# cmusatyalab/mega-nerf-viewer

Hardware: AMD Instinct MI355X
Metric: Mrays/sec at 1920x1080 on depth-10 SH-9 N3Tree; max|dRGBA| vs ref (higher is better)
Workload: dtype f32; 1 GPU; cfg2: depth-10 SH9 shell N3Tree (1,499,569 chunks), 1920x1080, 16-pose orbit per step x 4 laps; kernel=accel, partition=none, reserved_cus=0, march_streams=1, root_period=0, full=False

## Files before the change

### mega-nerf-viewer_amd/csrc/mnv_device.h

```cpp
#pragma once

#include <hip/hip_runtime.h>
#include <stdint.h>

#pragma clang fp contract(off)

namespace mnv {

struct __attribute__((aligned(16))) CamBlock {
    float fx, fy, cx, cy;
    float c2w[12];
    float cen[3];
    float pad;
};

struct FrameParams {
    CamBlock cam;
    int32_t x0, y0, tw, th;
    float offset[3], scale[3];
    float step_size, sigma_thresh, stop_thresh, background_brightness;
    float render_bbox[6];
    int32_t basis_min, basis_max;
    int32_t render_depth;
    int32_t rot_enabled;
    float rot_k[3], rot_cos, rot_sin;
    float *rgba;
    uint8_t *rgba8;
    const float *tmax_px;
    const uint8_t *rgba8_init;
};

__device__ __forceinline__ float frame_tmax(const FrameParams &P, int64_t p) { return P.tmax_px ? P.tmax_px[p] : 1e9f; }

struct MarchParams : FrameParams {
    const uint16_t *data;
    const int32_t *child;
    const int16_t *sample_counts;
    int32_t data_dim, basis_dim, format, capacity;
    int32_t max_depth, max_sample_count;
    float *split_track;
    float *sample_track;
    int32_t *visited;
    int32_t track_visit;
    int32_t N;
};

__device__ static const uint64_t kExp2fTab[32] = {
    0x3ff0000000000000ULL, 0x3fefd9b0d3158574ULL, 0x3fefb5586cf9890fULL, 0x3fef9301d0125b51ULL,
    0x3fef72b83c7d517bULL, 0x3fef54873168b9aaULL, 0x3fef387a6e756238ULL, 0x3fef1e9df51fdee1ULL,
    0x3fef06fe0a31b715ULL, 0x3feef1a7373aa9cbULL, 0x3feedea64c123422ULL, 0x3feece086061892dULL,
    0x3feebfdad5362a27ULL, 0x3feeb42b569d4f82ULL, 0x3feeab07dd485429ULL, 0x3feea47eb03a5585ULL,
    0x3feea09e667f3bcdULL, 0x3fee9f75e8ec5f74ULL, 0x3feea11473eb0187ULL, 0x3feea589994cce13ULL,
    0x3feeace5422aa0dbULL, 0x3feeb737b0cdc5e5ULL, 0x3feec49182a3f090ULL, 0x3feed503b23e255dULL,
    0x3feee89f995ad3adULL, 0x3feeff76f2fb5e47ULL, 0x3fef199bdd85529cULL, 0x3fef3720dcef9069ULL,
    0x3fef5818dcfba487ULL, 0x3fef7c97337b9b5fULL, 0x3fefa4afa2a490daULL, 0x3fefd0765b6e4540ULL,
};

__device__ __forceinline__ void load_exp_table(uint64_t *lds_tab) {
    if (threadIdx.x < 32) lds_tab[threadIdx.x] = kExp2fTab[threadIdx.x];
    __syncthreads();
}

__device__ __forceinline__ double expf_poly(double r, double c0, double c1, double c2) {
    double z, y;
    asm("v_fma_f64 %0, %1, %2, %3" : "=v"(z) : "s"(c0), "v"(r), "v"(c1));
    asm("v_fma_f64 %0, %1, %2, %3" : "=v"(y) : "v"(z), "v"(r), "s"(c2));
    return __builtin_fma(y, r, 1.0);
}

__device__ __forceinline__ float exact_expf(float x, const uint64_t *tab) {
    const uint32_t ix = __float_as_uint(x);
    const uint32_t abstop = (ix >> 20) & 0x7ffu;
    if (abstop >= 0x42bu) {
        if (ix == 0xff800000u) return 0.0f;
        if (abstop >= 0x7f8u) return x + x;
        if (x > 0x1.62e42ep6f) return __uint_as_float(0x7f800000u);
        if (x < -0x1.9fe368p6f) return 0.0f;
    }
    constexpr double N = 32.0;
    constexpr double InvLn2N = 0x1.71547652b82fep+0 * N;
    constexpr double SHIFT = 0x1.8p+52;
    constexpr double C0 = 0x1.c6af84b912394p-5 / N / N / N;
    constexpr double C1 = 0x1.ebfce50fac4f3p-3 / N / N;
    constexpr double C2 = 0x1.62e42ff0c52d6p-1 / N;
    const double xd = (double)x;
    double z = InvLn2N * xd;
    double kd = z + SHIFT;
    const uint64_t ki = (uint64_t)__double_as_longlong(kd);
    kd -= SHIFT;
    const double r = z - kd;
    uint64_t t = tab[ki & 31u];
    t += ki << 47;
    const double s = __longlong_as_double((long long)t);
    double y = expf_poly(r, C0, C1, C2);
    y = y * s;
    return (float)y;
}

__device__ __forceinline__ bool exact_expf_core_in_range(uint32_t abs_bits) { return abs_bits < 0x42b00000u; }
__device__ __forceinline__ float exact_expf_core(float x, const uint64_t *tab) {
    constexpr double N = 32.0;
    constexpr double InvLn2N = 0x1.71547652b82fep+0 * N;
    constexpr double SHIFT = 0x1.8p+52;
    constexpr double C0 = 0x1.c6af84b912394p-5 / N / N / N;
    constexpr double C1 = 0x1.ebfce50fac4f3p-3 / N / N;
    constexpr double C2 = 0x1.62e42ff0c52d6p-1 / N;
    const double xd = (double)x;
    double z = InvLn2N * xd;
    double kd = z + SHIFT;
    const uint64_t ki = (uint64_t)__double_as_longlong(kd);
    kd -= SHIFT;
    const double r = z - kd;
    uint64_t t = tab[ki & 31u];
    t += ki << 47;
    const double s = __longlong_as_double((long long)t);
    double y = expf_poly(r, C0, C1, C2);
    y = y * s;
    return (float)y;
}

__device__ __forceinline__ float exact_expf_select(float x, const uint64_t *tab) {
    constexpr double N = 32.0;
    constexpr double InvLn2N = 0x1.71547652b82fep+0 * N;
    constexpr double SHIFT = 0x1.8p+52;
    constexpr double C0 = 0x1.c6af84b912394p-5 / N / N / N;
    constexpr double C1 = 0x1.ebfce50fac4f3p-3 / N / N;
    constexpr double C2 = 0x1.62e42ff0c52d6p-1 / N;
    const float xc = __builtin_amdgcn_fmed3f(x, -128.f, 128.f);
    const double xd = (double)xc;
    double z = InvLn2N * xd;
    double kd = z + SHIFT;
    const uint64_t ki = (uint64_t)__double_as_longlong(kd);
    kd -= SHIFT;
    const double r = z - kd;
    uint64_t t = tab[ki & 31u];
    t += ki << 47;
    const double s = __longlong_as_double((long long)t);
    double y = expf_poly(r, C0, C1, C2);
    y = y * s;
    float res = (float)y;
    const uint32_t ix = __float_as_uint(x);
    const uint32_t abstop = (ix >> 20) & 0x7ffu;
    const bool big = abstop >= 0x42bu;
    res = (big && x < -0x1.9fe368p6f) ? 0.0f : res;
    res = (big && x > 0x1.62e42ep6f) ? __uint_as_float(0x7f800000u) : res;
    res = (big && abstop >= 0x7f8u) ? x + x : res;
    res = ix == 0xff800000u ? 0.0f : res;
    return res;
}

template <bool FAST>
__device__ __forceinline__ float colour_sigmoid(float w, float tmp, const uint64_t *s_exp) {
    if constexpr (FAST) {
        const float x = tmp * -1.44269504088896341f;
        const bool big = x > 96.f;
        const float e = __builtin_amdgcn_exp2f(big ? x - 64.f : x);
        const float den = __builtin_ldexpf((big ? 0x1p-64f : 1.f) + e, -32);
        return __builtin_ldexpf(w * __builtin_amdgcn_rcpf(den), big ? -96 : -32);
    } else {
        return w / (1.f + exact_expf(-tmp, s_exp));
    }
}

__device__ __forceinline__ float half_bits_to_float(uint16_t h) {
    _Float16 v;
    __builtin_memcpy(&v, &h, 2);
    return (float)v;
}

template <int BASIS>
__device__ __forceinline__ void sh_basis(const float vdir[3], float *out) {
    out[0] = (float)0.28209479177387814;
    if constexpr (BASIS >= 4) {
        const float x = vdir[0], y = vdir[1], z = vdir[2];
        const float xx = x * x, yy = y * y, zz = z * z;
        const float xy = x * y, yz = y * z, xz = x * z;
        if constexpr (BASIS >= 25) {
            out[16] = (float)(2.5033429417967046 * xy * (xx - yy));
            out[17] = (float)(-1.7701307697799304 * yz * (3 * xx - yy));
            out[18] = (float)(0.9461746957575601 * xy * (7 * zz - 1.f));
            out[19] = (float)(-0.6690465435572892 * yz * (7 * zz - 3.f));
            out[20] = (float)(0.10578554691520431 * (zz * (35 * zz - 30) + 3));
            out[21] = (float)(-0.6690465435572892 * xz * (7 * zz - 3));
            out[22] = (float)(0.47308734787878004 * (xx - yy) * (7 * zz - 1.f));
            out[23] = (float)(-1.7701307697799304 * xz * (xx - 3 * yy));
            out[24] = (float)(0.6258357354491761 * (xx * (xx - 3 * yy) - yy * (3 * xx - yy)));
        }
        if constexpr (BASIS >= 16) {
            out[9] = (float)(-0.5900435899266435 * y * (3 * xx - yy));
            out[10] = (float)(2.890611442640554 * xy * z);
            out[11] = (float)(-0.4570457994644658 * y * (4 * zz - xx - yy));
            out[12] = (float)(0.3731763325901154 * z * (2 * zz - 3 * xx - 3 * yy));
            out[13] = (float)(-0.4570457994644658 * x * (4 * zz - xx - yy));
            out[14] = (float)(1.445305721320277 * z * (xx - yy));
            out[15] = (float)(-0.5900435899266435 * x * (xx - 3 * yy));
        }
        if constexpr (BASIS >= 9) {
            out[4] = (float)(1.0925484305920792 * xy);
            out[5] = (float)(-1.0925484305920792 * yz);
            out[6] = (float)(0.31539156525252005 * (2.0 * zz - xx - yy));
            out[7] = (float)(-1.0925484305920792 * xz);
            out[8] = (float)(0.5462742152960396 * (xx - yy));
        }
        out[1] = (float)(-0.4886025119029199 * y);
        out[2] = (float)(0.4886025119029199 * z);
        out[3] = (float)(-0.4886025119029199 * x);
    }
}

__device__ __forceinline__ void world_ray_dirs(const FrameParams &P, const CamBlock &C, int ix, int iy, float true_dir[3], float vdir[3]) {
    const float *m = C.c2w;
    const float xyz0 = (ix + 0.5f - C.cx) / C.fx, xyz1 = -(iy + 0.5f - C.cy) / C.fy, xyz2 = -1.0f;
    true_dir[0] = m[0] * xyz0 + m[3] * xyz1 + m[6] * xyz2;
    true_dir[1] = m[1] * xyz0 + m[4] * xyz1 + m[7] * xyz2;
    true_dir[2] = m[2] * xyz0 + m[5] * xyz1 + m[8] * xyz2;
    const float inv = 1.f / sqrtf(true_dir[0] * true_dir[0] + true_dir[1] * true_dir[1] + true_dir[2] * true_dir[2]);
    for (int i = 0; i < 3; ++i) {
        true_dir[i] *= inv;
        vdir[i] = true_dir[i];
    }
    if (P.rot_enabled) {
        const float *k = P.rot_k;
        float cross[3];
        cross[0] = k[1] * vdir[2] - k[2] * vdir[1];
        cross[1] = k[2] * vdir[0] - k[0] * vdir[2];
        cross[2] = k[0] * vdir[1] - k[1] * vdir[0];
        const float dot = k[0] * vdir[0] + k[1] * vdir[1] + k[2] * vdir[2];
        for (int i = 0; i < 3; ++i)
            vdir[i] = (float)((double)(vdir[i] * P.rot_cos + cross[i] * P.rot_sin) + (double)(k[i] * dot) * (1.0 - (double)P.rot_cos));
    }
}

template <int NB>
struct RaySetup {
    float dir[3];
    float invdir[3];
    float basis[NB];
    float delta_scale;
    float tmin, tmax;
    bool in_bbox;
};

template <int BASIS>
__device__ __forceinline__ void setup_ray(const FrameParams &P, const CamBlock &C, int ix, int iy,
                                          RaySetup<(BASIS > 0 ? BASIS : 1)> &r, float t_max = 1e9f) {
    const float xyz0 = (ix + 0.5f - C.cx) / C.fx;
    const float xyz1 = -(iy + 0.5f - C.cy) / C.fy;
    const float xyz2 = -1.0f;
    const float *m = C.c2w;
    float dir[3];
    dir[0] = m[0] * xyz0 + m[3] * xyz1 + m[6] * xyz2;
    dir[1] = m[1] * xyz0 + m[4] * xyz1 + m[7] * xyz2;
    dir[2] = m[2] * xyz0 + m[5] * xyz1 + m[8] * xyz2;
    const float invnorm = 1.f / sqrtf(dir[0] * dir[0] + dir[1] * dir[1] + dir[2] * dir[2]);
    dir[0] *= invnorm;
    dir[1] *= invnorm;
    dir[2] *= invnorm;

    float vdir[3] = {dir[0], dir[1], dir[2]};
    if (P.rot_enabled) {
        const float *k = P.rot_k;
        float cross[3];
        cross[0] = k[1] * vdir[2] - k[2] * vdir[1];
        cross[1] = k[2] * vdir[0] - k[0] * vdir[2];
        cross[2] = k[0] * vdir[1] - k[1] * vdir[0];
        const float dot = k[0] * vdir[0] + k[1] * vdir[1] + k[2] * vdir[2];
#pragma unroll
        for (int i = 0; i < 3; ++i) {
            vdir[i] = (float)((double)(vdir[i] * P.rot_cos + cross[i] * P.rot_sin) +
                              (double)(k[i] * dot) * (1.0 - (double)P.rot_cos));
        }
    }

    dir[0] *= P.scale[0];
    dir[1] *= P.scale[1];
    dir[2] *= P.scale[2];
    const float delta_scale = 1.f / sqrtf(dir[0] * dir[0] + dir[1] * dir[1] + dir[2] * dir[2]);
    dir[0] *= delta_scale;
    dir[1] *= delta_scale;
    dir[2] *= delta_scale;
    r.delta_scale = delta_scale;
    const float tmax_bg = t_max / delta_scale;

    float tmin = 0.0f, tmax = 1e4f;
#pragma unroll
    for (int i = 0; i < 3; ++i) {
        r.dir[i] = dir[i];
        r.invdir[i] = (float)(1.0 / ((double)dir[i] + 1e-9));
        const double inv = (double)r.invdir[i];
        const float t1 = (float)(((double)P.render_bbox[i] + 1e-6 - (double)C.cen[i]) * inv);
        const float t2 = (float)(((double)P.render_bbox[i + 3] - 1e-6 - (double)C.cen[i]) * inv);
        tmin = fmaxf(tmin, fminf(t1, t2));
        tmax = fminf(tmax, fmaxf(t1, t2));
    }
    tmax = fminf(tmax, tmax_bg);
    r.tmin = tmin;
    r.tmax = tmax;
    r.in_bbox = !(tmax < 0 || tmin > tmax);

    constexpr int NB = (BASIS > 0 ? BASIS : 1);
    if constexpr (BASIS > 0) {
        sh_basis<BASIS>(vdir, r.basis);
#pragma unroll
        for (int i = 0; i < NB; ++i)
            if (i < P.basis_min || i > P.basis_max) r.basis[i] = 0.f;
    } else {
        r.basis[0] = 0.f;
    }
}

template <int BASIS>
__device__ __forceinline__ void setup_ray_dir(const FrameParams &P, const float (&cen)[3], float (&dir)[3],
                                              RaySetup<(BASIS > 0 ? BASIS : 1)> &r, float t_max) {
    const float invnorm = 1.f / sqrtf(dir[0] * dir[0] + dir[1] * dir[1] + dir[2] * dir[2]);
    dir[0] *= invnorm;
    dir[1] *= invnorm;
    dir[2] *= invnorm;

    float vdir[3] = {dir[0], dir[1], dir[2]};
    if (P.rot_enabled) {
        const float *k = P.rot_k;
        float cross[3];
        cross[0] = k[1] * vdir[2] - k[2] * vdir[1];
        cross[1] = k[2] * vdir[0] - k[0] * vdir[2];
        cross[2] = k[0] * vdir[1] - k[1] * vdir[0];
        const float dot = k[0] * vdir[0] + k[1] * vdir[1] + k[2] * vdir[2];
#pragma unroll
        for (int i = 0; i < 3; ++i) {
            vdir[i] = (float)((double)(vdir[i] * P.rot_cos + cross[i] * P.rot_sin) +
                              (double)(k[i] * dot) * (1.0 - (double)P.rot_cos));
        }
    }

    dir[0] *= P.scale[0];
    dir[1] *= P.scale[1];
    dir[2] *= P.scale[2];
    const float delta_scale = 1.f / sqrtf(dir[0] * dir[0] + dir[1] * dir[1] + dir[2] * dir[2]);
    dir[0] *= delta_scale;
    dir[1] *= delta_scale;
    dir[2] *= delta_scale;
    r.delta_scale = delta_scale;
    const float tmax_bg = t_max / delta_scale;

    float tmin = 0.0f, tmax = 1e4f;
#pragma unroll
    for (int i = 0; i < 3; ++i) {
        r.dir[i] = dir[i];
        r.invdir[i] = (float)(1.0 / ((double)dir[i] + 1e-9));
        const double inv = (double)r.invdir[i];
        const float t1 = (float)(((double)P.render_bbox[i] + 1e-6 - (double)cen[i]) * inv);
        const float t2 = (float)(((double)P.render_bbox[i + 3] - 1e-6 - (double)cen[i]) * inv);
        tmin = fmaxf(tmin, fminf(t1, t2));
        tmax = fminf(tmax, fmaxf(t1, t2));
    }
    tmax = fminf(tmax, tmax_bg);
    r.tmin = tmin;
    r.tmax = tmax;
    r.in_bbox = !(tmax < 0 || tmin > tmax);

    constexpr int NB = (BASIS > 0 ? BASIS : 1);
    if constexpr (BASIS > 0) {
        sh_basis<BASIS>(vdir, r.basis);
#pragma unroll
        for (int i = 0; i < NB; ++i)
            if (i < P.basis_min || i > P.basis_max) r.basis[i] = 0.f;
    } else {
        r.basis[0] = 0.f;
    }
}

template <int BASIS, typename F>
__device__ __forceinline__ float sh_channel(const float *b, F coef, int off) {
    float tmp = b[0] * coef(off);
    if constexpr (BASIS >= 25) {
        tmp += b[16] * coef(off + 16) + b[17] * coef(off + 17) + b[18] * coef(off + 18) +
               b[19] * coef(off + 19) + b[20] * coef(off + 20) + b[21] * coef(off + 21) +
               b[22] * coef(off + 22) + b[23] * coef(off + 23) + b[24] * coef(off + 24);
    }
    if constexpr (BASIS >= 16) {
        tmp += b[9] * coef(off + 9) + b[10] * coef(off + 10) + b[11] * coef(off + 11) +
               b[12] * coef(off + 12) + b[13] * coef(off + 13) + b[14] * coef(off + 14) +
               b[15] * coef(off + 15);
    }
    if constexpr (BASIS >= 9) {
        tmp += b[4] * coef(off + 4) + b[5] * coef(off + 5) + b[6] * coef(off + 6) + b[7] * coef(off + 7) +
               b[8] * coef(off + 8);
    }
    if constexpr (BASIS >= 4) {
        tmp += b[1] * coef(off + 1) + b[2] * coef(off + 2) + b[3] * coef(off + 3);
    }
    return tmp;
}

__device__ __forceinline__ float half_mul(uint32_t word, bool hi, float b) {
    float r;
    if (hi) asm("v_fma_mix_f32 %0, %1, %2, neg(0) op_sel:[1,0,0] op_sel_hi:[1,0,0]" : "=v"(r) : "v"(word), "v"(b));
    else asm("v_fma_mix_f32 %0, %1, %2, neg(0) op_sel_hi:[1,0,0]" : "=v"(r) : "v"(word), "v"(b));
    return r;
}

template <int BASIS, typename W>
__device__ __forceinline__ float sh_channel_mix(const float *b, W word, int off) {
    auto p = [&](int k) -> float { return half_mul(word((off + k) >> 1), ((off + k) & 1) != 0, b[k]); };
    float tmp = p(0);
    if constexpr (BASIS >= 25) {
        tmp += p(16) + p(17) + p(18) + p(19) + p(20) + p(21) + p(22) + p(23) + p(24);
    }
    if constexpr (BASIS >= 16) {
        tmp += p(9) + p(10) + p(11) + p(12) + p(13) + p(14) + p(15);
    }
    if constexpr (BASIS >= 9) {
        tmp += p(4) + p(5) + p(6) + p(7) + p(8);
    }
    if constexpr (BASIS >= 4) {
        tmp += p(1) + p(2) + p(3);
    }
    return tmp;
}

__device__ __forceinline__ uint32_t pack_u8(float v) {
    const float s = v * 255.f;
    if (!(s > 0.f)) return 0u;
    if (s >= 255.f) return 255u;
    return (uint32_t)s;
}

__device__ __forceinline__ void composite_and_write(const FrameParams &P, int64_t p, float o0, float o1,
                                                    float o2, float o3) {
    const float nalpha = 1.f - o3;
    if (P.rgba8_init) {
        const uint32_t px = reinterpret_cast<const uint32_t *>(P.rgba8_init)[p];
        o0 += (float)(int)(px & 0xffu) / 255.f * nalpha;
        o1 += (float)(int)((px >> 8) & 0xffu) / 255.f * nalpha;
        o2 += (float)(int)((px >> 16) & 0xffu) / 255.f * nalpha;
    } else {
        const float remain = P.background_brightness * nalpha;
        o0 += remain;
        o1 += remain;
        o2 += remain;
    }
    if (P.rgba) reinterpret_cast<float4 *>(P.rgba)[p] = make_float4(o0, o1, o2, o3);
    if (P.rgba8)
        reinterpret_cast<uint32_t *>(P.rgba8)[p] =
            pack_u8(o0) | (pack_u8(o1) << 8) | (pack_u8(o2) << 16) | (255u << 24);
}

}
```

### mega-nerf-viewer_amd/csrc/mnv_march_accel_kernel.h

```cpp
#pragma once

#include "mnv_march_diag.h"

#pragma clang fp contract(off)

namespace mnv {

enum : int { kShapeGeneric = 0, kShapeL3G9 = 1, kShapeL3G9Recs = 2 };
constexpr int kShapeLdsLevel = 3, kShapeGrid2Level = 9;

template <int BASIS, int BLOCK, int MODE ,
          bool BRICK = false ,
          bool RAYS = false ,
          int SHAPE = kShapeGeneric >
#if defined(MNV_NUM_VGPR) && defined(MNV_NUM_SGPR)
#define MNV_EXTRA_KERNEL_ATTR __attribute__((amdgpu_num_vgpr(MNV_NUM_VGPR), amdgpu_num_sgpr(MNV_NUM_SGPR)))
#elif defined(MNV_NUM_VGPR)
#define MNV_EXTRA_KERNEL_ATTR __attribute__((amdgpu_num_vgpr(MNV_NUM_VGPR)))
#else
#define MNV_EXTRA_KERNEL_ATTR
#endif
__global__ __launch_bounds__(BLOCK, (MODE == 2 || MODE == 3) ? MNV_TRACK_WAVES : RAYS ? MNV_RAY_WAVES : MNV_MIN_WAVES) MNV_EXTRA_KERNEL_ATTR void march_accel_kernel(const LaunchBlock<RAYS> K) {
    extern __shared__ __attribute__((aligned(16))) uint32_t s_mem[];
    uint64_t *s_exp = reinterpret_cast<uint64_t *>(s_mem);
    constexpr int NB = BASIS > 0 ? BASIS : 1;
    auto depth_mode = [&]() -> bool {
        if constexpr (MODE == 0 || MODE == 4) return false;
        else if constexpr (MODE == 5) return true;
        else return K.P.render_depth != 0;
    };
    constexpr int MAPW = BASIS >= 16 ? BLOCK : 0;
    uint32_t *s_map = s_mem + 64;
    float *s_ray = reinterpret_cast<float *>(s_mem + 64 + MAPW);
    constexpr int RAY_ROWS = NB + 2 + ((MODE == 2 || MODE == 3) ? 1 : 0);
    uint32_t *s_grid = s_mem + 64 + MAPW + RAY_ROWS * BLOCK;
    constexpr int CHAN_BYTES = chan_bytes_for(BASIS);
    constexpr int ROW_BYTES = row_bytes_pow2(BASIS);
    const FrameParams &P = K.P;
    const AccelView &A = K.A;

    static_assert(SHAPE == kShapeGeneric || (BRICK && !RAYS && (MODE == 0 || MODE == 4)), "fixed lookup shapes: plain colour frames on inline cell words only");
    constexpr bool FIXED = SHAPE != kShapeGeneric;
    const int LL = FIXED ? kShapeLdsLevel : K.lds_level;
    const int cells = 1 << (3 * LL);
    if (threadIdx.x < 32) s_exp[threadIdx.x] = kExp2fTab[threadIdx.x];
    if (LL == A.grid_level) {
        for (int i = threadIdx.x; i < cells; i += BLOCK) s_grid[i] = A.grid[i];
    } else {
        for (int i = threadIdx.x; i < cells; i += BLOCK) {
            const int G = 1 << LL;
            const int iz = i & (G - 1), iy = (i >> LL) & (G - 1), ix = i >> (2 * LL);
            uint32_t chunk = 0, word = 0;
            for (int l = 1; l <= LL; ++l) {
                const int s = LL - l;
                const int cidx = (((ix >> s) & 1) << 2) | (((iy >> s) & 1) << 1) | ((iz >> s) & 1);
                word = A.nodes[(int64_t)chunk * 8 + cidx];
                if (word & kLeafBit) break;
                chunk = word;
            }
            s_grid[i] = word;
        }
    }
    __syncthreads();

    const int lane = threadIdx.x & 63;
    const int Lq = FIXED ? 23 : A.max_depth;
    const float qscale = FIXED ? 8388608.f : __uint_as_float((uint32_t)(127 + Lq) << 23);
    const int sh1 = Lq - LL;
    const int L2 = FIXED ? kShapeGrid2Level : A.grid2_level;
    const int sh2 = Lq - L2;
    const int shg = Lq - A.grid_level;
    float *my_ray = s_ray + threadIdx.x;
    float *wave_ray = s_ray + (threadIdx.x & ~63);

    const CamBlock *__restrict__ Cp = K.cams;
    float cen0 = 0.f, cen1 = 0.f, cen2 = 0.f;
    if constexpr (!RAYS) {
        cen0 = Cp->cen[0];
        cen1 = Cp->cen[1];
        cen2 = Cp->cen[2];
    }
    float t = 0.f, T = 1.f, o0 = 0.f, o1 = 0.f, o2 = 0.f;
    float dir0 = 0.f, dir1 = 0.f, dir2 = 0.f, inv0 = 0.f, inv1 = 0.f, inv2 = 0.f, tmax = 0.f;
    bool alive = false;
    float max_weight = -1.f, max_sample_weight = -1.f, sp_prio = 0.f, sa_prio = 0.f;
    int32_t sp_vox = -1, sa_vox = -1;
    int32_t ns = 0;
    [[maybe_unused]] float sp_t = -1.f, sa_t = -1.f;
    [[maybe_unused]] auto leaf_at = [&](float tw, uint32_t &word, uint32_t &v, float &dt) {
        float pos[3];
        uint32_t q[3];
        pos[0] = cen0 + tw * dir0;
        pos[1] = cen1 + tw * dir1;
        pos[2] = cen2 + tw * dir2;
#pragma unroll
        for (int i = 0; i < 3; ++i) {
            pos[i] = __builtin_amdgcn_fmed3f(pos[i], 0.f, 1.f - 1e-6f);
            q[i] = (uint32_t)(pos[i] * qscale);
        }
        word = s_grid[((((q[0] >> sh1) << LL) | (q[1] >> sh1)) << LL) | (q[2] >> sh1)];
        int src = 0;
        v = 0;
        if (!(word & kLeafBit)) word = descend_to_leaf(A, q, word, sh1, sh2, L2, LL, src, v);
        if (src == 0) v = A.grid_vox[((((q[0] >> shg) << A.grid_level) + (q[1] >> shg)) << A.grid_level) + (q[2] >> shg)];
        else if (src == 1) v = A.grid2_vox[v];
        const int depth = (int)((word >> 16) & 0x7fu);
        const float sc = __uint_as_float((uint32_t)(127 + depth) << 23), inv_cube = __uint_as_float((uint32_t)(127 - depth) << 23);
        const float invd[3] = {inv0, inv1, inv2};
        float tu = 1e4f;
#pragma unroll
        for (int i = 0; i < 3; ++i) {
            const float x = __builtin_amdgcn_fractf(pos[i] * sc);
            const float t1 = -x * invd[i];
            const float t2 = t1 + invd[i];
            tu = fminf(tu, fmaxf(t1, t2));
        }
        dt = tu * inv_cube + P.step_size;
    };
    [[maybe_unused]] auto resolve_fallbacks = [&]() {
        if constexpr (MODE == 2 || MODE == 3) {
            const bool want_split = max_weight == -1.f && sp_t >= 0.f, want_sample = K.sample_counts && max_sample_weight == -1.f && sa_t >= 0.f;
            uint32_t word = 0, v = 0;
            float dt = 0.f;
            if (want_split) {
                leaf_at(sp_t, word, v, dt);
                sp_vox = (int32_t)v;
                sp_prio = (float)((word >> 16) & 0x7fu);
            }
            if (want_sample) {
                if (!(want_split && sa_t == sp_t)) leaf_at(sa_t, word, v, dt);
                const int16_t sc_last = K.sample_counts[v];
                if (sc_last < K.max_sample_count) {
                    sa_vox = (int32_t)v;
                    sa_prio = (float)sc_last;
                } else {
                    float tw = my_ray[(NB + 2) * BLOCK];
                    while (tw < t) {
                        leaf_at(tw, word, v, dt);
                        if (!(half_bits_to_float((uint16_t)word) > P.sigma_thresh)) {
                            const int16_t c = K.sample_counts[v];
                            if (c < K.max_sample_count) {
                                sa_vox = (int32_t)v;
                                sa_prio = (float)c;
                            }
                        }
                        tw += dt;
                    }
                }
            }
        }
    };
    auto write_trackers = [&](uint32_t p) {
        resolve_fallbacks();
        if constexpr (MODE == 3) K.num_samples[p] = (int16_t)ns;
        if constexpr (MODE == 2 || MODE == 3) {
            if (K.split_track) {
                K.split_track[(int64_t)p * 3 + 0] = sp_prio;
                K.split_track[(int64_t)p * 3 + 1] = sp_vox < 0 ? -1.f : (float)(sp_vox >> 3);
                K.split_track[(int64_t)p * 3 + 2] = sp_vox < 0 ? -1.f : (float)(sp_vox & 7);
            }
            if (K.sample_track) {
                K.sample_track[(int64_t)p * 3 + 0] = sa_prio;
                K.sample_track[(int64_t)p * 3 + 1] = sa_vox < 0 ? -1.f : (float)(sa_vox >> 3);
                K.sample_track[(int64_t)p * 3 + 2] = sa_vox < 0 ? -1.f : (float)(sa_vox & 7);
            }
        }
    };

    int fin = 0;
    auto flush_finished = [&]() {
        if (fin != 0) {
            float a;
            if (fin == 3) {
                o0 = o1 = o2 = 0.f;
                a = depth_mode() ? 1.f : 0.f;
            } else if (fin == 1) {
                a = 1.f - T;
                if (depth_mode()) {
                    o0 = o1 = o2 = fminf(o0 * 0.3f, 1.0f);
                    a = 1.f;
                }
            } else {
                if (depth_mode()) o0 = o1 = o2 = fminf(o0 * 0.3f, 1.0f);
                const float sc = 1.f / (1.f - T);
                o0 *= sc;
                o1 *= sc;
                o2 *= sc;
                a = 1.f;
            }
            const uint32_t p = __float_as_uint(my_ray[(NB + 1) * BLOCK]);
            if constexpr (MODE != 3) composite_and_write(P, (int64_t)p, o0, o1, o2, a);
            write_trackers(p);
            fin = 0;
        }
    };

    const uint32_t home = blockIdx.x % kNumQueues;
    uint32_t qsel = 0;
    bool drained = false;
    uint32_t frame = 0;
    uint32_t pix_base = 0;

    MarchProbe<MODE, RAYS, BLOCK> probe(K, lane);
    probe.wave_begin();

    for (;;) {
        const uint64_t idle = __ballot(!alive);
        const int n_idle = __popcll(idle);
        probe.count(kCountOuterIter, true);
        probe.iteration();
        if (!drained && n_idle >= K.refill_min) {
            flush_finished();
            if (qsel >= kNumQueues) {
                drained = true;
            } else {
            const uint32_t q = (home + qsel) % kNumQueues;
            const uint32_t begin = K.band_begin[q] * 64u, span = (K.band_begin[q + 1] - K.band_begin[q]) * 64u;
            const uint32_t grab = (uint32_t)n_idle;
            uint32_t off = 0;
            if (lane == 0) off = atomicAdd(&K.queue[q * 16], grab);
            off = __builtin_amdgcn_readfirstlane(off);
            if (span == 0 || (uint64_t)off >= (uint64_t)span * K.n_frames) {
                ++qsel;
                continue;
            }
            uint32_t f = 0;
            if (K.n_frames > 1) {
                f = off / span;
                off -= f * span;
                if (f != frame) {
                    frame = f;
                    Cp = K.cams + f;
                    cen0 = Cp->cen[0];
                    cen1 = Cp->cen[1];
                    cen2 = Cp->cen[2];
                    pix_base = f * K.frame_stride_px;
                }
            }
            const uint32_t base = begin + off, end = begin + span;
            probe.tile_grabbed(f, base);
            if (!alive) {
                const uint32_t rank = __builtin_amdgcn_mbcnt_hi((uint32_t)(idle >> 32), __builtin_amdgcn_mbcnt_lo((uint32_t)idle, 0u));
                const uint32_t id = base + rank;
                if (rank < grab && id < end) {
                    int bx, by;
                    probe.count(kCountRefill, true);
                    uint32_t pix;
                    if (ray_pixel(K, id, bx, by, pix)) {
                        pix += pix_base;
                        if constexpr (MODE == 2 || MODE == 3) {
                            max_weight = max_sample_weight = -1.f;
                            sp_prio = (float)(K.max_depth + 1);
                            sa_prio = (float)(K.max_sample_count + 1);
                            sp_vox = sa_vox = -1;
                            sp_t = sa_t = -1.f;
                        }
                        if constexpr (MODE == 3) ns = K.num_samples[pix];
                        RaySetup<NB> r;
                        if constexpr (RAYS) {
                            const float *__restrict__ ro = K.ray_origins + (int64_t)pix * 3, *__restrict__ rd = K.ray_dirs + (int64_t)pix * 3;
                            const float w0 = ro[0], w1 = ro[1], w2 = ro[2];
                            float d[3] = {rd[0], rd[1], rd[2]};
                            const float len2 = d[0] * d[0] + d[1] * d[1] + d[2] * d[2];
                            const bool valid = len2 > 0.f && len2 < __builtin_inff() && (w0 - w0) + (w1 - w1) + (w2 - w2) == 0.f;
                            const float p0 = P.scale[0] * w0, p1 = P.scale[1] * w1, p2 = P.scale[2] * w2;
                            const float cen[3] = {P.offset[0] + p0, P.offset[1] + p1, P.offset[2] + p2};
                            setup_ray_dir<(BASIS > 0 ? BASIS : 0)>(P, cen, d, r, frame_tmax(P, pix));
                            r.in_bbox = r.in_bbox && valid;
                            cen0 = cen[0];
                            cen1 = cen[1];
                            cen2 = cen[2];
                        } else {
                            setup_ray<(BASIS > 0 ? BASIS : 0)>(P, *Cp, P.x0 + bx, P.y0 + by, r, frame_tmax(P, pix));
                        }
                        if constexpr (BASIS == 0)
                            r.basis[0] = (0 < P.basis_min || 0 > P.basis_max) ? 0.f : (float)0.28209479177387814;
                        o0 = o1 = o2 = 0.f;
                        if (r.in_bbox) {
                            alive = true;
                            t = r.tmin;
                            T = 1.f;
                            tmax = r.tmax;
                            dir0 = r.dir[0]; dir1 = r.dir[1]; dir2 = r.dir[2];
                            inv0 = r.invdir[0]; inv1 = r.invdir[1]; inv2 = r.invdir[2];
                            if constexpr (MODE == 3) {
                                float true_dir[3], vdir[3];
                                world_ray_dirs(P, *Cp, P.x0 + bx, P.y0 + by, true_dir, vdir);
#pragma unroll
                                for (int k = 0; k < 3; ++k) {
                                    my_ray[k * BLOCK] = true_dir[k];
                                    my_ray[(3 + k) * BLOCK] = vdir[k];
                                }
                            } else {
#pragma unroll
                                for (int k = 0; k < NB; ++k) my_ray[k * BLOCK] = r.basis[k];
                            }
                            my_ray[NB * BLOCK] = r.delta_scale;
                            my_ray[(NB + 1) * BLOCK] = __uint_as_float(pix);
                            if constexpr (MODE == 2 || MODE == 3) my_ray[(NB + 2) * BLOCK] = r.tmin;
                        } else {
                            my_ray[(NB + 1) * BLOCK] = __uint_as_float(pix);
                            fin = 3;
                        }
                    }
                }
            }
            }
        }
        if (__ballot(alive) == 0) {
            probe.tile_done();
            if (drained) {
                flush_finished();
                break;
            }
            continue;
        }
        bool dense = false;
        [[maybe_unused]] bool cand = false;
        [[maybe_unused]] float sigma_held = 0.f;
        float delta_t = 0.f, weight = 0.f, att = 1.f;
        uint32_t vox = 0;
        [[maybe_unused]] bool track_leaf = false;
        [[maybe_unused]] int track_depth = 0;
        [[maybe_unused]] auto track_update = [&]() {
            if constexpr (MODE == 2 || MODE == 3) {
                if (track_leaf) {
                    if (dense) {
                        if (track_depth < K.max_depth && weight > max_weight) {
                            sp_vox = (int32_t)vox;
                            sp_prio = (float)track_depth;
                            max_weight = weight;
                        }
                        if (K.sample_counts && weight > max_sample_weight) {
                            const int16_t sc = K.sample_counts[vox];
                            if (sc < K.max_sample_count) {
                                sa_vox = (int32_t)vox;
                                sa_prio = (float)sc;
                                max_sample_weight = weight;
                            }
                        }
                    } else {
                        if (max_weight == -1.f && track_depth < K.max_depth) sp_t = t;
                        if (max_sample_weight == -1.f) sa_t = t;
                    }
                }
            }
        };
        probe.step_begin();
        if (alive) {
            if (!(t < tmax)) {
                fin = 1;
                alive = false;
            } else {
                probe.count(kCountMarchStep, true);
                float pos[3];
                uint32_t q[3];
                pos[0] = cen0 + t * dir0;
                pos[1] = cen1 + t * dir1;
                pos[2] = cen2 + t * dir2;
#pragma unroll
                for (int i = 0; i < 3; ++i) {
                    pos[i] = __builtin_amdgcn_fmed3f(pos[i], 0.f, 1.f - 1e-6f);
                    q[i] = (uint32_t)(pos[i] * qscale);
                }
                uint32_t word = s_grid[((((q[0] >> sh1) << LL) | (q[1] >> sh1)) << LL) | (q[2] >> sh1)];
                int src = 0;
                if (!(word & kLeafBit)) {
                    int sh = sh1;
                    if (L2 > LL) {
                        const int LB = L2 - 2;
                        uint32_t g = q[0] >> (sh2 + 2);
                        g = (g << LB) | (q[1] >> (sh2 + 2));
                        g = (g << LB) | (q[2] >> (sh2 + 2));
                        g = (g << 2) | __builtin_amdgcn_ubfe(q[0], (uint32_t)sh2, 2u);
                        g = (g << 2) | __builtin_amdgcn_ubfe(q[1], (uint32_t)sh2, 2u);
                        vox = (g << 2) | __builtin_amdgcn_ubfe(q[2], (uint32_t)sh2, 2u);
                        if constexpr (BRICK) word = A.grid2i[vox];
                        else word = A.grid2[vox];
                        probe.touch(kLinesGrid2, (uint64_t)vox * 4);
                        src = 1;
                        sh = sh2;
                        if constexpr ((kShadow & 8) != 0) shadow_load(A.grid2_vox + vox);
                        if constexpr (BRICK) {
                            if (!(word & kLeafBit)) {
                                uint32_t s1 = __builtin_amdgcn_ubfe(q[0], (uint32_t)(sh2 - 1), 1u);
                                s1 = (s1 << 1) | __builtin_amdgcn_ubfe(q[1], (uint32_t)(sh2 - 1), 1u);
                                s1 = (s1 << 1) | __builtin_amdgcn_ubfe(q[2], (uint32_t)(sh2 - 1), 1u);
                                if (word & kInlineBit) {
                                    vox = (((word & ((1u << kInlineMaskShift) - 1u)) + A.inline_base) << 3) | s1;
                                    cand = ((word >> (kInlineMaskShift + s1)) & 1u) != 0u;
                                    word = kLeafBit | ((uint32_t)(L2 + 1) << 16);
                                    src = 2;
                                }
                            }
                            if (SHAPE != kShapeL3G9 && !(word & kLeafBit) && (SHAPE == kShapeL3G9Recs || A.recs != nullptr)) {
                                probe.count(kCountNodeLoad, true);
                                uint32_t s1 = __builtin_amdgcn_ubfe(q[0], (uint32_t)(sh2 - 1), 1u), s2 = __builtin_amdgcn_ubfe(q[0], (uint32_t)(sh2 - 2), 1u);
                                s1 = (s1 << 1) | __builtin_amdgcn_ubfe(q[1], (uint32_t)(sh2 - 1), 1u);
                                s2 = (s2 << 1) | __builtin_amdgcn_ubfe(q[1], (uint32_t)(sh2 - 2), 1u);
                                s1 = (s1 << 1) | __builtin_amdgcn_ubfe(q[2], (uint32_t)(sh2 - 1), 1u);
                                s2 = (s2 << 1) | __builtin_amdgcn_ubfe(q[2], (uint32_t)(sh2 - 2), 1u);
                                const uint2 e = A.recs[(int64_t)word * 8 + s1];
                                probe.touch(kLinesRecs, ((uint64_t)word * 8 + s1) * 8);
                                if constexpr ((kShadow & 64) != 0) shadow_load(K.shadow_recs + ((int64_t)word * 8 + s1));
                                const uint32_t code = __builtin_amdgcn_ubfe(e.y, s2 << 1, 2u);
                                vox = code == 1u ? ((word << 3) | s1) : ((e.x << 3) | s2);
                                cand = code == 3u;
                                word = code != 0u ? (kLeafBit | ((uint32_t)(L2 + 2 - (code == 1u ? 1 : 0)) << 16)) : word;
                                src = 2;
                            }
                        }
                    }
                    while (!(word & kLeafBit)) {
                        probe.count(kCountNodeLoad, true);
                        --sh;
                        uint32_t v = (word << 1) | __builtin_amdgcn_ubfe(q[0], (uint32_t)sh, 1u);
                        v = (v << 1) | __builtin_amdgcn_ubfe(q[1], (uint32_t)sh, 1u);
                        vox = (v << 1) | __builtin_amdgcn_ubfe(q[2], (uint32_t)sh, 1u);
                        word = A.nodes[vox];
                        probe.touch(kLinesNodes, (uint64_t)vox * 4);
                        src = 2;
                        if constexpr ((kShadow & 16) != 0) shadow_load(K.shadow_nodes + vox);
                    }
                }
                if constexpr (BRICK && MODE == 3) {
                    if (cand) {
                        word = A.nodes[vox];
                        cand = false;
                    }
                }
                probe.template phase_end<kPhaseLookup>();
                const int depth = (int)((word >> 16) & 0x7fu);
                const float sc = __uint_as_float((uint32_t)(127 + depth) << 23);
                const float inv_cube = __uint_as_float((uint32_t)(127 - depth) << 23);
                float tu = 1e4f;
                const float invd[3] = {inv0, inv1, inv2};
#pragma unroll
                for (int i = 0; i < 3; ++i) {
                    const float x = __builtin_amdgcn_fractf(pos[i] * sc);
                    const float t1 = -x * invd[i];
                    const float t2 = t1 + invd[i];
                    tu = fminf(tu, fmaxf(t1, t2));
                }
                delta_t = tu * inv_cube + P.step_size;
                const float sigma = half_bits_to_float((uint16_t)word);
                const bool is_dense = sigma > P.sigma_thresh && !probe.ablate(2);
                bool need_vox = is_dense;
                if constexpr (MODE == 2 || MODE == 3) need_vox = is_dense || cand || K.visited != nullptr;
                if (need_vox) {
                    if (src == 0) {
                        const uint32_t gc = ((((q[0] >> shg) << A.grid_level) + (q[1] >> shg)) << A.grid_level) + (q[2] >> shg);
                        vox = A.grid_vox[gc];
                        probe.touch(kLinesGridVox, (uint64_t)gc * 4);
                    } else if (src == 1) {
                        probe.touch(kLinesGrid2Vox, (uint64_t)vox * 4);
                        vox = A.grid2_vox[vox];
                    }
                }
                if constexpr (MODE == 2 || MODE == 3) {
                    if (K.visited && __hip_atomic_load(&K.visited[vox >> 3], __ATOMIC_RELAXED, __HIP_MEMORY_SCOPE_AGENT) == 0) K.visited[vox >> 3] = 1;
                }
                if constexpr (BRICK && MODE != 3) {
                    dense = (is_dense || cand) && !probe.ablate(2);
                    sigma_held = sigma;
                } else if (is_dense) {
                    dense = true;
                    att = exact_expf(-delta_t * my_ray[NB * BLOCK] * sigma, s_exp);
                    weight = T * (1.f - att);
                }
                if constexpr (MODE == 2 || MODE == 3) {
                    track_leaf = true;
                    track_depth = depth;
                    if constexpr (!(BRICK && MODE == 2)) track_update();
                }
                if constexpr (MODE == 3) {
                    if (is_dense && ns < K.max_guided_samples) {
                        const uint32_t p = __float_as_uint(my_ray[(NB + 1) * BLOCK]);
                        float *row = K.samples + ((int64_t)p * K.max_guided_samples + ns) * K.samples_dim;
                        const float tz0 = t * dir0 / P.scale[0], tz1 = t * dir1 / P.scale[1], tz2 = t * dir2 / P.scale[2];
                        const float z = sqrtf(tz0 * tz0 + tz1 * tz1 + tz2 * tz2);
                        const float *m = Cp->c2w;
                        const float wx = m[9] + my_ray[0 * BLOCK] * z, wy = m[10] + my_ray[1 * BLOCK] * z, wz = m[11] + my_ray[2 * BLOCK] * z;
                        row[0] = z;
                        row[1] = wx;
                        row[2] = wy;
                        row[3] = wz;
                        if (K.need_viewdir) {
                            row[4] = my_ray[3 * BLOCK];
                            row[5] = my_ray[4 * BLOCK];
                            row[6] = my_ray[5 * BLOCK];
                            if (K.appearance_embedding != -1) row[7] = (float)K.appearance_embedding;
                        } else if (K.appearance_embedding != -1) {
                            row[4] = (float)K.appearance_embedding;
                        }
                        const int g1 = (int)fmaxf(fminf((wy - K.min_position[1]) / K.range[1] * (float)K.grid_dim[0], (float)K.grid_dim[0] - 1.0f), 0.0f);
                        const int g2 = (int)fmaxf(fminf((wz - K.min_position[2]) / K.range[2] * (float)K.grid_dim[1], (float)K.grid_dim[1] - 1.0f), 0.0f);
                        K.cluster_indices[(int64_t)p * K.max_guided_samples + ns] = (int16_t)(g1 * K.grid_dim[1] + g2);
                        ns += 1;
                    }
                }
            }
        }
        probe.template phase_end<kPhaseStep>();
        const uint64_t dense_mask = __ballot(dense);
        if (dense_mask != 0) {
            probe.count(kCountDense, dense);
            [[maybe_unused]] auto settle = [&](uint32_t row_sigma_bits) {
                const float sg = cand ? half_bits_to_float((uint16_t)row_sigma_bits) : sigma_held;
                if (sg > P.sigma_thresh) {
                    att = exact_expf(-delta_t * my_ray[NB * BLOCK] * sg, s_exp);
                    weight = T * (1.f - att);
                } else {
                    dense = false;
                }
            };
            [[maybe_unused]] auto settle_from_memory = [&]() {
                if constexpr (BRICK) {
                    if (dense && cand) probe.touch(kLinesRows, (uint64_t)vox * A.row_bytes + A.sigma_off);
                    if (dense) settle(cand ? (uint32_t)*reinterpret_cast<const uint16_t *>(A.rows + (int64_t)vox * A.row_bytes + A.sigma_off) : 0u);
                }
            };
            if constexpr (MODE == 3) {
            } else if (depth_mode()) {
                settle_from_memory();
                if (dense) o0 += weight * t;
            } else if (probe.ablate(1)) {
                settle_from_memory();
            } else if constexpr (BASIS >= 16) {
                const int n_dense = __popcll(dense_mask);
                const int rank = (int)__builtin_amdgcn_mbcnt_hi((uint32_t)(dense_mask >> 32), __builtin_amdgcn_mbcnt_lo((uint32_t)dense_mask, 0u));
                uint32_t *map = s_map + (threadIdx.x & ~63);
                if (dense) map[rank] = (uint32_t)lane;
                __builtin_amdgcn_wave_barrier();
                const int my_s = lane / 3, my_c = lane - 3 * my_s;
                for (int base = 0; base < n_dense; base += 21) {
                    const int smp = base + my_s;
                    const bool task = my_s < 21 && smp < n_dense;
                    probe.count(kCountColourPass, task);
                    const int owner = task ? (int)map[smp] : lane;
                    const float w = lane_read(weight, owner);
                    uint32_t vx = lane_read(vox, owner);
                    if (probe.ablate(4)) vx &= 0xffffu;
                    float b[NB];
#pragma unroll
                    for (int k = 0; k < NB; ++k) b[k] = wave_ray[k * BLOCK + owner];
                    float v = 0.f;
                    if (task) {
                        constexpr int NW = CHAN_BYTES / 4;
                        ChanWords<NW> cw;
                        cw = *reinterpret_cast<const ChanWords<NW> *>(A.rows + (int64_t)vx * ROW_BYTES + my_c * CHAN_BYTES);
                        const float tmp = sh_channel_mix<BASIS>(b, [&](int j) -> uint32_t { return cw.w[j]; }, 0);
                        v = colour_sigmoid<MODE == 4>(w, tmp, s_exp);
                    }
                    const int rl = rank - base;
                    const bool mine = dense && rl >= 0 && rl < 21;
                    const int from = mine ? 3 * rl : lane;
                    const float v0 = lane_read(v, from), v1 = lane_read(v, mine ? from + 1 : lane), v2 = lane_read(v, mine ? from + 2 : lane);
                    if (mine) {
                        o0 += v0;
                        o1 += v1;
                        o2 += v2;
                    }
                }
                __builtin_amdgcn_wave_barrier();
            } else if constexpr (BASIS >= 1) {
                if (dense) {
                    probe.count(kCountColourPass, true);
                    uint32_t vx = vox;
                    if (probe.ablate(4)) vx &= 0xffffu;
                    const uint8_t *row = A.rows + (int64_t)vx * ROW_BYTES;
                    probe.touch(kLinesRows, (uint64_t)vx * ROW_BYTES);
                    if constexpr ((kShadow & 32) != 0) shadow_load(reinterpret_cast<const uint32_t *>(K.shadow_rows + (int64_t)vx * ROW_BYTES));
                    constexpr int RW = ROW_BYTES / 4;
                    uint32_t rw[RW];
                    if constexpr (RW >= 4) {
#pragma unroll
                        for (int u = 0; u < RW / 4; ++u) {
                            const uint4 x = reinterpret_cast<const uint4 *>(row)[u];
                            rw[4 * u] = x.x;
                            rw[4 * u + 1] = x.y;
                            rw[4 * u + 2] = x.z;
                            rw[4 * u + 3] = x.w;
                        }
                    } else {
                        const uint2 x = *reinterpret_cast<const uint2 *>(row);
                        rw[0] = x.x;
                        rw[1] = x.y;
                    }
                    probe.template phase_end<kPhaseRow>();
                    auto half_at = [&](int hidx) -> uint32_t { return (hidx & 1) ? (rw[hidx >> 1] >> 16) : (rw[hidx >> 1] & 0xffffu); };
                    if constexpr (BRICK && !RAYS && MODE != 4) {
                        float b[NB];
#pragma unroll
                        for (int k = 0; k < NB; ++k) b[k] = my_ray[k * BLOCK];
                        const float sg = cand ? half_bits_to_float((uint16_t)half_at(3 * BASIS)) : sigma_held;
                        if (!(sg > P.sigma_thresh)) dense = false;
                        const float a0 = -delta_t * my_ray[NB * BLOCK] * sg;
                        const float t0 = sh_channel_mix<BASIS>(b, [&](int j) -> uint32_t { return rw[j]; }, 0);
                        const float t1 = sh_channel_mix<BASIS>(b, [&](int j) -> uint32_t { return rw[j]; }, BASIS);
                        const float t2 = sh_channel_mix<BASIS>(b, [&](int j) -> uint32_t { return rw[j]; }, 2 * BASIS);
                        constexpr uint32_t kAbs = 0x7fffffffu;
                        const uint32_t m = max(max(__float_as_uint(a0) & kAbs, __float_as_uint(t0) & kAbs), max(__float_as_uint(t1) & kAbs, __float_as_uint(t2) & kAbs));
                        float e0, e1, e2;
                        const bool all_in_range = __ballot(dense && !exact_expf_core_in_range(m)) == 0;
                        if (all_in_range) {
                            probe.count(kCountExpUniform, dense);
                            att = exact_expf_core(a0, s_exp);
                            e0 = exact_expf_core(-t0, s_exp);
                            e1 = exact_expf_core(-t1, s_exp);
                            e2 = exact_expf_core(-t2, s_exp);
                        } else {
                            probe.count(kCountExpGeneral, dense);
                            att = exact_expf(a0, s_exp);
                            e0 = exact_expf(-t0, s_exp);
                            e1 = exact_expf(-t1, s_exp);
                            e2 = exact_expf(-t2, s_exp);
                        }
                        if (dense) {
                            weight = T * (1.f - att);
                            o0 += weight / (1.f + e0);
                            o1 += weight / (1.f + e1);
                            o2 += weight / (1.f + e2);
                        }
                    } else {
                        if constexpr (BRICK) settle(half_at(3 * BASIS));
                        float b[NB];
#pragma unroll
                        for (int k = 0; k < NB; ++k) b[k] = my_ray[k * BLOCK];
                        auto chan = [&](int c) -> float {
                            const float tmp = sh_channel_mix<BASIS>(b, [&](int j) -> uint32_t { return rw[j]; }, c * BASIS);
                            return colour_sigmoid<MODE == 4>(weight, tmp, s_exp);
                        };
                        if (dense) {
                            o0 += chan(0);
                            o1 += chan(1);
                            o2 += chan(2);
                        }
                    }
                }
            } else {
                if (dense) {
                    const uint2 qd = *reinterpret_cast<const uint2 *>(A.rows + (int64_t)vox * ROW_BYTES);
                    if constexpr (BRICK) settle(qd.y >> 16);
                    if (dense) {
                        o0 += half_mul(qd.x, false, weight);
                        o1 += half_mul(qd.x, true, weight);
                        o2 += half_mul(qd.y, false, weight);
                    }
                }
            }
            if constexpr (BRICK && MODE == 2) track_update();
            if (dense) {
                T *= att;
                if (T < P.stop_thresh) {
                    fin = 2;
                    alive = false;
                }
            }
        }
        if constexpr (BRICK && MODE == 2) {
            if (dense_mask == 0) track_update();
        }
        t += delta_t;
        probe.template phase_end<kPhaseColour>();
    }
    probe.wave_end();
}

}
```

Measured before the change: 9985 Mrays/s.

## Add inner march loop that skips refill checks while enough lanes stay alive

For brick, non-ray-list kernels in modes 0 and 4, the march step now runs inside an inner do-while loop. The loop keeps stepping until the number of live lanes drops to the refill threshold, so the outer ballot, refill and flush logic no longer runs every step. The t-advance moves earlier in the step and the termination check is hoisted. It also reworks the expf scale construction to do 32-bit arithmetic on the high dword, and pins some setup_ray params to SGPRs with empty asm to shape codegen. The risk is a different register allocation and changed loop structure.

Result: faster. 10480 Mrays/s, median of 6 (+4.9%).

```diff
diff --git a/mega-nerf-viewer_amd/csrc/mnv_device.h b/mega-nerf-viewer_amd/csrc/mnv_device.h
--- a/mega-nerf-viewer_amd/csrc/mnv_device.h
+++ b/mega-nerf-viewer_amd/csrc/mnv_device.h
@@ -111,9 +111,10 @@
     const uint64_t ki = (uint64_t)__double_as_longlong(kd);
     kd -= SHIFT;
     const double r = z - kd;
-    uint64_t t = tab[ki & 31u];
-    t += ki << 47;
-    const double s = __longlong_as_double((long long)t);
+    typedef uint32_t dwords __attribute__((ext_vector_type(2)));
+    dwords t = __builtin_bit_cast(dwords, tab[ki & 31u]);
+    t.y += (uint32_t)ki << 15;
+    const double s = __builtin_bit_cast(double, t);
     double y = expf_poly(r, C0, C1, C2);
     y = y * s;
     return (float)y;
@@ -241,9 +242,13 @@
     bool in_bbox;
 };
 
-template <int BASIS>
+template <int BASIS, bool FRESH = false>
 __device__ __forceinline__ void setup_ray(const FrameParams &P, const CamBlock &C, int ix, int iy,
                                           RaySetup<(BASIS > 0 ? BASIS : 1)> &r, float t_max = 1e9f) {
+    auto fresh = [](float x) -> float {
+        if constexpr (FRESH) asm volatile("" : "+s"(x));
+        return x;
+    };
     const float xyz0 = (ix + 0.5f - C.cx) / C.fx;
     const float xyz1 = -(iy + 0.5f - C.cy) / C.fy;
     const float xyz2 = -1.0f;
@@ -268,7 +273,7 @@
 #pragma unroll
         for (int i = 0; i < 3; ++i) {
             vdir[i] = (float)((double)(vdir[i] * P.rot_cos + cross[i] * P.rot_sin) +
-                              (double)(k[i] * dot) * (1.0 - (double)P.rot_cos));
+                              (double)(k[i] * dot) * (1.0 - (double)fresh(P.rot_cos)));
         }
     }
 
@@ -288,8 +293,8 @@
         r.dir[i] = dir[i];
         r.invdir[i] = (float)(1.0 / ((double)dir[i] + 1e-9));
         const double inv = (double)r.invdir[i];
-        const float t1 = (float)(((double)P.render_bbox[i] + 1e-6 - (double)C.cen[i]) * inv);
-        const float t2 = (float)(((double)P.render_bbox[i + 3] - 1e-6 - (double)C.cen[i]) * inv);
+        const float t1 = (float)(((double)fresh(P.render_bbox[i]) + 1e-6 - (double)C.cen[i]) * inv);
+        const float t2 = (float)(((double)fresh(P.render_bbox[i + 3]) - 1e-6 - (double)C.cen[i]) * inv);
         tmin = fmaxf(tmin, fminf(t1, t2));
         tmax = fminf(tmax, fmaxf(t1, t2));
     }
diff --git a/mega-nerf-viewer_amd/csrc/mnv_march_accel_kernel.h b/mega-nerf-viewer_amd/csrc/mnv_march_accel_kernel.h
--- a/mega-nerf-viewer_amd/csrc/mnv_march_accel_kernel.h
+++ b/mega-nerf-viewer_amd/csrc/mnv_march_accel_kernel.h
@@ -204,6 +204,7 @@
     MarchProbe<MODE, RAYS, BLOCK> probe(K, lane);
     probe.wave_begin();
 
+    constexpr bool INNER = BRICK && !RAYS && (MODE == 0 || MODE == 4);
     for (;;) {
         const uint64_t idle = __ballot(!alive);
         const int n_idle = __popcll(idle);
@@ -271,7 +272,7 @@
                             cen1 = cen[1];
                             cen2 = cen[2];
                         } else {
-                            setup_ray<(BASIS > 0 ? BASIS : 0)>(P, *Cp, P.x0 + bx, P.y0 + by, r, frame_tmax(P, pix));
+                            setup_ray<(BASIS > 0 ? BASIS : 0), INNER>(P, *Cp, P.x0 + bx, P.y0 + by, r, frame_tmax(P, pix));
                         }
                         if constexpr (BASIS == 0)
                             r.basis[0] = (0 < P.basis_min || 0 > P.basis_max) ? 0.f : (float)0.28209479177387814;
@@ -315,6 +316,9 @@
             }
             continue;
         }
+        [[maybe_unused]] const int stay_above = (!INNER || drained) ? 0 : max(64 - (int)K.refill_min, 0);
+        [[maybe_unused]] uint64_t live = 0;
+        do {
         bool dense = false;
         [[maybe_unused]] bool cand = false;
         [[maybe_unused]] float sigma_held = 0.f;
@@ -347,8 +351,14 @@
             }
         };
         probe.step_begin();
+        if constexpr (INNER) {
+            if (alive && !(t < tmax)) {
+                fin = 1;
+                alive = false;
+            }
+        }
         if (alive) {
-            if (!(t < tmax)) {
+            if (!INNER && !(t < tmax)) {
                 fin = 1;
                 alive = false;
             } else {
@@ -443,6 +453,7 @@
                     tu = fminf(tu, fmaxf(t1, t2));
                 }
                 delta_t = tu * inv_cube + P.step_size;
+                if constexpr (INNER) t += delta_t;
                 const float sigma = half_bits_to_float((uint16_t)word);
                 const bool is_dense = sigma > P.sigma_thresh && !probe.ablate(2);
                 bool need_vox = is_dense;
@@ -661,8 +672,10 @@
         if constexpr (BRICK && MODE == 2) {
             if (dense_mask == 0) track_update();
         }
-        t += delta_t;
+        if constexpr (!INNER) t += delta_t;
         probe.template phase_end<kPhaseColour>();
+        if constexpr (INNER) live = __ballot(alive);
+        } while (INNER && __popcll(live) > stay_above);
     }
     probe.wave_end();
 }
```
